# suutari/meterelf

Hardware: AMD Instinct MI355X
Metric: frames/sec (640x480), full pipeline, digits identical to the oracle (higher is better)
Workload: dtype u8; 1 GPU; Batch=1024 per GPU, full pipeline incl. TM_CCOEFF match + needle reading, 4 dials/frame, sample-images1 params, frames 480x640 synthesised from the readable fixtures (shift +-8, noise sigma 2), 4 distinct batches in rotation (3.77 GB of frames per GPU); global_batch=1024, parallelism=dp1, frames_read_ok_batch0=1023

## Files before the change

meterelf_amd/csrc/k_dials.hip:

```cpp
#include <limits.h>
#include <stdlib.h>

#include "melf_device.h"
#include "melf_internal.h"

namespace melf {

__device__ inline double py_fmod(double a, double b)
{
    double m = fmod(a, b);
    if (m != 0.0) {
        if ((b < 0) != (m < 0)) m += b;
    } else {
        m = copysign(0.0, b);
    }
    return m;
}

__device__ inline bool angle_by_vector(double x, double y, double& out)
{
    if (y == 0) {
        if (x > 0) { out = 0.25; return true; }
        if (x < 0) { out = 0.75; return true; }
        return false;
    }
    const double at = atan(x / y) / (2 * 3.141592653589793);
    const double v = -at + (y > 0 ? 0.5 : 0.0);
    double m = v - trunc(v);
    if (m != 0.0) { if (m < 0) m += 1.0; } else { m = 0.0; }
    out = m;
    return true;
}

__device__ inline double value_by_positions(double r4, double r3, double r2, double r1)
{
    int d3 = (int)r3 + ((py_fmod(r3, 1.0) > 0.55 && r4 <= 2) ? 1 : 0) - ((py_fmod(r3, 1.0) < 0.45 && r4 >= 8) ? 1 : 0);
    d3 = ((d3 % 10) + 10) % 10;
    int d2 = (int)r2 + ((py_fmod(r2, 1.0) > 0.55 && d3 <= 2) ? 1 : 0) - ((py_fmod(r2, 1.0) < 0.45 && d3 >= 8) ? 1 : 0);
    d2 = ((d2 % 10) + 10) % 10;
    int d1 = (int)r1 + ((py_fmod(r1, 1.0) > 0.55 && d2 <= 2) ? 1 : 0) - ((py_fmod(r1, 1.0) < 0.45 && d2 >= 8) ? 1 : 0);
    d1 = ((d1 % 10) + 10) % 10;
    return (d1 * 100.0) + (d2 * 10.0) + (d3 * 1.0) + r4 / 10.0;
}

struct Key {
    double a, d;
};
__device__ inline bool key_lt(const Key& p, const Key& q) { return p.a < q.a || (p.a == q.a && p.d < q.d); }
__device__ inline void wave_min_max_key(const Key& lo, const Key& hi, Key& klo, Key& khi)
{
    klo.a = wave_min_f64(lo.a);
    khi.a = wave_max_f64(hi.a);
    const uint64_t blo = __builtin_amdgcn_ballot_w64(lo.a == klo.a), bhi = __builtin_amdgcn_ballot_w64(hi.a == khi.a);
    if (__popcll(blo) == 1 && __popcll(bhi) == 1) {
        const int jl = __builtin_ctzll(blo), jh = __builtin_ctzll(bhi);
        const uint64_t dl = __double_as_longlong(lo.d), dh = __double_as_longlong(hi.d);
        klo.d = __longlong_as_double((uint64_t)(uint32_t)__builtin_amdgcn_readlane((int)(uint32_t)dl, jl) |
                                     ((uint64_t)(uint32_t)__builtin_amdgcn_readlane((int)(uint32_t)(dl >> 32), jl) << 32));
        khi.d = __longlong_as_double((uint64_t)(uint32_t)__builtin_amdgcn_readlane((int)(uint32_t)dh, jh) |
                                     ((uint64_t)(uint32_t)__builtin_amdgcn_readlane((int)(uint32_t)(dh >> 32), jh) << 32));
    } else {
        klo.d = wave_min_f64(lo.a == klo.a ? lo.d : 1e300);
        khi.d = wave_max_f64(hi.a == khi.a ? hi.d : -1e300);
    }
}

template <class F>
__device__ inline void for_each_kept(uint64_t outer, int lane, int wx0, int wy0, double cx, double cy,
                                     bool have_mom, double mom, F&& fn)
{
    const double dy = (double)(wy0 + lane) - cy;
    uint64_t bits = outer;
    while (bits) {
        const int x = __builtin_ctzll(bits);
        bits &= bits - 1;
        const double dx = (double)(wx0 + x) - cx;
        double a;
        if (angle_by_vector(dx, dy, a) && have_mom) {
            double dist = fabs(a - mom);
            const double dist2 = fabs(fabs(a - mom) - 1);
            if (dist2 < dist) dist = dist2;
            if (dist < 0.25) fn(a, dx * dx + dy * dy);
        }
    }
}

constexpr int DIAL_LIST_CAP = 768;
constexpr int RING_CAP = 512;
constexpr int RING_CAP_REGS = 1024;
constexpr int DIAL_LDS_BYTES = 5120;
static_assert(DIAL_LIST_CAP * 4 + DIAL_LIST_CAP * 2 <= 4608 && RING_CAP * 8 + RING_CAP * 2 <= DIAL_LDS_BYTES, "dial LDS layout");

__device__ __forceinline__ uint32_t load_px3(const uint8_t* p, const uint8_t* buffer_start)
{
    const uint32_t back = p == buffer_start ? 0u : 1u;
    uint32_t v;
    __builtin_memcpy(&v, p - back, 4);
    return v >> (8u * back);
}

struct PxColumn {
    const uint8_t* first;
    uint32_t shift;
};
__device__ __forceinline__ PxColumn px_column(const uint8_t* col, const uint8_t* buffer_start)
{
    const bool at_start = col == buffer_start;
    return PxColumn{at_start ? col : col - 1, at_start ? 0u : 8u};
}
__device__ __forceinline__ uint32_t load_px3_row(const PxColumn& c, size_t row_off)
{
    asm("" : "+s"(row_off));
    uint32_t v;
    __builtin_memcpy(&v, c.first + row_off, 4);
    return v >> c.shift;
}

typedef unsigned short u16x2v __attribute__((ext_vector_type(2)));
typedef uint32_t u32x4v __attribute__((ext_vector_type(4)));
__device__ __forceinline__ uint32_t pk_max_u16(uint32_t a, uint32_t b)
{
    return __builtin_bit_cast(uint32_t, __builtin_elementwise_max(__builtin_bit_cast(u16x2v, a), __builtin_bit_cast(u16x2v, b)));
}
__device__ __forceinline__ uint32_t pk_min_u16(uint32_t a, uint32_t b)
{
    return __builtin_bit_cast(uint32_t, __builtin_elementwise_min(__builtin_bit_cast(u16x2v, a), __builtin_bit_cast(u16x2v, b)));
}
__device__ __forceinline__ uint32_t pk_add_u16(uint32_t a, uint32_t b)
{
    return __builtin_bit_cast(uint32_t, (u16x2v)(__builtin_bit_cast(u16x2v, a) + __builtin_bit_cast(u16x2v, b)));
}
__device__ __forceinline__ uint32_t pk_sub_u16(uint32_t a, uint32_t b)
{
    return __builtin_bit_cast(uint32_t, (u16x2v)(__builtin_bit_cast(u16x2v, a) - __builtin_bit_cast(u16x2v, b)));
}
__device__ __forceinline__ uint32_t pk_mul_u16(uint32_t a, uint32_t b)
{
    return __builtin_bit_cast(uint32_t, (u16x2v)(__builtin_bit_cast(u16x2v, a) * __builtin_bit_cast(u16x2v, b)));
}

__device__ __forceinline__ void write_record(melf_result* __restrict__ out, int lane, int status, int mx, int my, float mv, int failed_dial,
                                             uint32_t unreadable, double value, double pos_lane, double angle_lane)
{
    if (lane < MELF_MAX_DIALS) {
        out->pos[lane] = pos_lane;
        out->angle[lane] = angle_lane;
    }
    if (lane == 0) {
        out->status = status;
        out->match_x = mx; out->match_y = my;
        out->failed_dial = failed_dial;
        out->unreadable_mask = unreadable;
        out->match_val = mv;
        out->value = value;
    }
}
static_assert(sizeof(melf_result) == 24 + 16 * MELF_MAX_DIALS + 8, "melf_result has padding: write_record must fill it");

#ifdef MELF_DIALS_STAMP
__device__ uint64_t g_dials_stamps[8 * 8192];
extern "C" __attribute__((visibility("default"))) int melf_debug_dials_stamps(uint64_t* out, int nwaves)
{
    return hipMemcpyFromSymbol(out, HIP_SYMBOL(g_dials_stamps), sizeof(uint64_t) * 8 * (size_t)(nwaves < 8192 ? nwaves : 8192)) == hipSuccess ? 0 : -1;
}
__device__ uint64_t g_dials_real[8 * 8192];
extern "C" __attribute__((visibility("default"))) int melf_debug_dials_real(uint64_t* out, int nwaves)
{
    return hipMemcpyFromSymbol(out, HIP_SYMBOL(g_dials_real), sizeof(uint64_t) * 8 * (size_t)(nwaves < 8192 ? nwaves : 8192)) == hipSuccess ? 0 : -1;
}
__device__ uint64_t g_dials_fine[16 * 8192];
extern "C" __attribute__((visibility("default"))) int melf_debug_dials_fine(uint64_t* out, int nwaves)
{
    return hipMemcpyFromSymbol(out, HIP_SYMBOL(g_dials_fine), sizeof(uint64_t) * 16 * (size_t)(nwaves < 8192 ? nwaves : 8192)) == hipSuccess ? 0 : -1;
}
#define FSTAMPD(k) do { if (lane == 0 && (int)(blockIdx.x * (blockDim.x >> 6) + wv) < 8192) g_dials_fine[16 * (blockIdx.x * (blockDim.x >> 6) + wv) + (k)] = __builtin_amdgcn_s_memtime(); } while (0)
#define DSTAMP(k) do { if (lane == 0 && (int)(blockIdx.x * (blockDim.x >> 6) + wv) < 8192) { \
        g_dials_stamps[8 * (blockIdx.x * (blockDim.x >> 6) + wv) + (k)] = __builtin_amdgcn_s_memtime(); \
        if ((k) < 6) g_dials_real[8 * (blockIdx.x * (blockDim.x >> 6) + wv) + (k)] = __builtin_amdgcn_s_memrealtime(); \
        if ((k) == 0) { uint32_t hw_; asm volatile("s_getreg_b32 %0, hwreg(HW_REG_HW_ID)" : "=s"(hw_)); uint32_t xc_; asm volatile("s_getreg_b32 %0, hwreg(HW_REG_XCC_ID)" : "=s"(xc_)); \
                        g_dials_real[8 * (blockIdx.x * (blockDim.x >> 6) + wv) + 6] = hw_; g_dials_real[8 * (blockIdx.x * (blockDim.x >> 6) + wv) + 7] = xc_ & 15u; } } } while (0)
#else
#define DSTAMP(k) do { } while (0)
#define FSTAMPD(k) do { } while (0)
#endif

constexpr int DIALS_VGPRS = 64;
template <int PB>
__device__ __forceinline__ uint32_t load_px(const uint8_t* p, const uint8_t* buffer_start)
{
    if constexpr (PB == 4) return *(const uint32_t*)p;
    else return load_px3(p, buffer_start);
}
template <int PB>
__device__ __forceinline__ PxColumn px_column_of(const uint8_t* col, const uint8_t* buffer_start)
{
    if constexpr (PB == 4) return PxColumn{col, 0u};
    else return px_column(col, buffer_start);
}

template <bool FROM_HLS, int NR>
__global__ __launch_bounds__(64 * MELF_MAX_DIALS, 4) __attribute__((amdgpu_num_vgpr(DIALS_VGPRS))) void k_dials(DialsSrc src, melf_params P,
                                                              const DialGeom* __restrict__ geom,
                                                              const uint64_t* __restrict__ rowmasks,
                                                              const MatchPartial* __restrict__ partials,
                                                              int nparts, int rw, melf_result* __restrict__ results)
{
    constexpr int PB = 3;
    constexpr bool RT_ORDER = false;
    const uint32_t bsel = 0u;
#include "k_dials_body.inc"
}

template <int BPP, int NR>
__global__ __launch_bounds__(64 * MELF_MAX_DIALS, 4) __attribute__((amdgpu_num_vgpr(DIALS_VGPRS))) void k_needles(DialsSrc src, melf_params P,
                                                                const DialGeom* __restrict__ geom,
                                                                const uint64_t* __restrict__ rowmasks,
                                                                const MatchPartial* __restrict__ partials,
                                                                int nparts, int rw, melf_result* __restrict__ results, int swap_rb)
{
    constexpr bool FROM_HLS = false;
    constexpr int PB = BPP;
    constexpr bool RT_ORDER = true;
    const uint32_t bsel = swap_rb ? 0x00020002u : 0u;
#include "k_dials_body.inc"
}

#define MELF_YUV_BODY
template <bool PLANAR, int NR>
__global__ __launch_bounds__(64 * MELF_MAX_DIALS, 4) __attribute__((amdgpu_num_vgpr(DIALS_VGPRS))) void k_yneedle(DialsSrc src, YuvPlanes yuv, YuvMatrix ymat, melf_params P,
                                                                const DialGeom* __restrict__ geom,
                                                                const uint64_t* __restrict__ rowmasks,
                                                                const MatchPartial* __restrict__ partials,
                                                                int nparts, int rw, melf_result* __restrict__ results)
{
    constexpr bool FROM_HLS = false;
    constexpr int PB = 4;
    constexpr bool RT_ORDER = false;
    const uint32_t bsel = 0u;
#include "k_dials_body.inc"
}
#undef MELF_YUV_BODY

#define MELF_P422_BODY
template <int NR>
__global__ __launch_bounds__(64 * MELF_MAX_DIALS, 4) __attribute__((amdgpu_num_vgpr(DIALS_VGPRS))) void k_p422_needle(DialsSrc src, uint32_t psel, YuvMatrix ymat, melf_params P,
                                                                const DialGeom* __restrict__ geom,
                                                                const uint64_t* __restrict__ rowmasks,
                                                                const MatchPartial* __restrict__ partials,
                                                                int nparts, int rw, melf_result* __restrict__ results)
{
    constexpr bool FROM_HLS = false;
    constexpr int PB = 4;
    constexpr bool RT_ORDER = false;
    const uint32_t bsel = 0u;
#include "k_dials_body.inc"
}
#undef MELF_P422_BODY

#define MELF_PLANAR_BODY
template <int NR>
__global__ __launch_bounds__(64 * MELF_MAX_DIALS, 4) __attribute__((amdgpu_num_vgpr(DIALS_VGPRS))) void k_planar_needle(DialsSrc src, PlanarPlanes planes, melf_params P,
                                                                const DialGeom* __restrict__ geom,
                                                                const uint64_t* __restrict__ rowmasks,
                                                                const MatchPartial* __restrict__ partials,
                                                                int nparts, int rw, melf_result* __restrict__ results)
{
    constexpr bool FROM_HLS = false;
    constexpr int PB = 4;
    constexpr bool RT_ORDER = false;
    const uint32_t bsel = 0u;
#include "k_dials_body.inc"
}
#undef MELF_PLANAR_BODY

void launch_dials(const DialsSrc& src, int pix, int n, const melf_params& P, const DialGeom* d_geom,
                  const uint64_t* d_rowmasks, const MatchPartial* d_partials, int nparts, int rw,
                  melf_result* d_results, hipStream_t stream, int ws_max, const YuvPlanes* yuv, const PlanarPlanes* planes,
                  const YuvMatrix* ymat)
{
    dim3 grid(n), block(64 * P.ndials);
    const size_t shmem = (size_t)P.ndials * DIAL_LDS_BYTES;
    const int nr = ws_max <= 32 ? 32 : (ws_max <= 40 ? 40 : (ws_max <= 48 ? 48 : (ws_max <= 52 ? 52 : (ws_max <= 56 ? 56 : 64))));
#define MELF_DIALS_LAUNCH(HLS, NRV) \
    hipLaunchKernelGGL((k_dials<HLS, NRV>), grid, block, shmem, stream, src, P, d_geom, d_rowmasks, d_partials, nparts, rw, d_results)
#define MELF_DIALS_NR(HLS)                                   \
    switch (nr) {                                            \
        case 32: MELF_DIALS_LAUNCH(HLS, 32); break;          \
        case 40: MELF_DIALS_LAUNCH(HLS, 40); break;          \
        case 48: MELF_DIALS_LAUNCH(HLS, 48); break;          \
        case 52: MELF_DIALS_LAUNCH(HLS, 52); break;          \
        case 56: MELF_DIALS_LAUNCH(HLS, 56); break;          \
        default: MELF_DIALS_LAUNCH(HLS, 64); break;          \
    }
#define MELF_NEEDLES_LAUNCH(BPP, NRV)                                                                                          \
    hipLaunchKernelGGL((k_needles<BPP, NRV>), grid, block, shmem, stream, src, P, d_geom, d_rowmasks, d_partials, nparts, rw, d_results, \
                       swap_rb)
#define MELF_NEEDLES_NR(BPP)                                 \
    switch (nr) {                                            \
        case 32: MELF_NEEDLES_LAUNCH(BPP, 32); break;        \
        case 40: MELF_NEEDLES_LAUNCH(BPP, 40); break;        \
        case 48: MELF_NEEDLES_LAUNCH(BPP, 48); break;        \
        case 52: MELF_NEEDLES_LAUNCH(BPP, 52); break;        \
        case 56: MELF_NEEDLES_LAUNCH(BPP, 56); break;        \
        default: MELF_NEEDLES_LAUNCH(BPP, 64); break;        \
    }
#define MELF_YNEEDLE_LAUNCH(PL, NRV) \
    hipLaunchKernelGGL((k_yneedle<PL, NRV>), grid, block, shmem, stream, src, *yuv, *ymat, P, d_geom, d_rowmasks, d_partials, nparts, rw, d_results)
#define MELF_YNEEDLE_NR(PL)                                  \
    switch (nr) {                                            \
        case 32: MELF_YNEEDLE_LAUNCH(PL, 32); break;         \
        case 40: MELF_YNEEDLE_LAUNCH(PL, 40); break;         \
        case 48: MELF_YNEEDLE_LAUNCH(PL, 48); break;         \
        case 52: MELF_YNEEDLE_LAUNCH(PL, 52); break;         \
        case 56: MELF_YNEEDLE_LAUNCH(PL, 56); break;         \
        default: MELF_YNEEDLE_LAUNCH(PL, 64); break;         \
    }
#define MELF_P422_NEEDLE_LAUNCH(NRV) \
    hipLaunchKernelGGL((k_p422_needle<NRV>), grid, block, shmem, stream, src, p422_sel(pix), *ymat, P, d_geom, d_rowmasks, d_partials, nparts, rw, d_results)
#define MELF_PLANAR_NEEDLE_LAUNCH(NRV) \
    hipLaunchKernelGGL((k_planar_needle<NRV>), grid, block, shmem, stream, src, *planes, P, d_geom, d_rowmasks, d_partials, nparts, rw, d_results)
    const int swap_rb = pix == MELF_PIX_RGB || pix == MELF_PIX_RGBA;
    if (pix == PIX_PLANAR) {
        switch (nr) {
            case 32: MELF_PLANAR_NEEDLE_LAUNCH(32); break;
            case 40: MELF_PLANAR_NEEDLE_LAUNCH(40); break;
            case 48: MELF_PLANAR_NEEDLE_LAUNCH(48); break;
            case 52: MELF_PLANAR_NEEDLE_LAUNCH(52); break;
            case 56: MELF_PLANAR_NEEDLE_LAUNCH(56); break;
            default: MELF_PLANAR_NEEDLE_LAUNCH(64); break;
        }
    }
    else if (pix_p422(pix)) {
        switch (nr) {
            case 32: MELF_P422_NEEDLE_LAUNCH(32); break;
            case 40: MELF_P422_NEEDLE_LAUNCH(40); break;
            case 48: MELF_P422_NEEDLE_LAUNCH(48); break;
            case 52: MELF_P422_NEEDLE_LAUNCH(52); break;
            case 56: MELF_P422_NEEDLE_LAUNCH(56); break;
            default: MELF_P422_NEEDLE_LAUNCH(64); break;
        }
    }
    else if (pix == PIX_NV12) { MELF_YNEEDLE_NR(false) }
    else if (pix == PIX_I420) { MELF_YNEEDLE_NR(true) }
    else if (pix == PIX_PLANE) { MELF_DIALS_NR(true) }
    else if (pix == MELF_PIX_BGR) { MELF_DIALS_NR(false) }
    else if (pix == MELF_PIX_RGB) { MELF_NEEDLES_NR(3) }
    else { MELF_NEEDLES_NR(4) }
#undef MELF_PLANAR_NEEDLE_LAUNCH
#undef MELF_P422_NEEDLE_LAUNCH
#undef MELF_YNEEDLE_NR
#undef MELF_YNEEDLE_LAUNCH
#undef MELF_NEEDLES_NR
#undef MELF_NEEDLES_LAUNCH
#undef MELF_DIALS_NR
#undef MELF_DIALS_LAUNCH
}

}
```

meterelf_amd/csrc/k_dials_body.inc:

```
    [[maybe_unused]] const uint32_t csel = bsel ? 0x0c000102u : 0x0c020100u;
    auto bgr = [&](uint32_t px) -> uint32_t {
        if constexpr (RT_ORDER) return __builtin_amdgcn_perm(0u, px, csel);
        else return px;
    };
    __shared__ int s_status[MELF_MAX_DIALS];
    __shared__ double s_pos[MELF_MAX_DIALS], s_angle[MELF_MAX_DIALS];
    extern __shared__ __attribute__((aligned(16))) uint8_t s_dyn[];

    const int f = blockIdx.x;
    const int lane = threadIdx.x & 63, wv = threadIdx.x >> 6;
    const int d = wv;
    DSTAMP(0);
    const uint8_t* frame = src.base + (size_t)f * src.frame_stride;
    uint8_t* const lds = s_dyn + (size_t)wv * DIAL_LDS_BYTES;
    uint32_t* const list_px = (uint32_t*)lds;
    uint16_t* const list_pos = (uint16_t*)(lds + 3072);
    double* const s_ra_d = (double*)lds;
    uint16_t* const ring_list = (uint16_t*)(lds + 4096);
    uint32_t* const mask_d = (uint32_t*)(lds + 4608);

    int mx = 0, my = 0;
    float mv = 0.f;
    if (!FROM_HLS) {
        float bv = 0.f;
        int bi = INT_MAX;
        for (int k = lane; k < nparts; k += 64) {
            const MatchPartial p = partials[(size_t)f * nparts + k];
            if (p.idx != INT_MAX && (bi == INT_MAX || p.val > bv || (p.val == bv && p.idx < bi))) { bv = p.val; bi = p.idx; }
        }
        {
            auto fold = [&](float ov, int oi) {
                if (oi != INT_MAX && (bi == INT_MAX || ov > bv || (ov == bv && oi < bi))) { bv = ov; bi = oi; }
            };
#define MELF_PFOLD(CTRL, RM, BM) \
            fold(__int_as_float(dpp_i32<CTRL, RM, BM>(0, __float_as_int(bv))), dpp_i32<CTRL, RM, BM>(INT_MAX, bi));
            MELF_PFOLD(0x111, 0xf, 0xf) MELF_PFOLD(0x112, 0xf, 0xf) MELF_PFOLD(0x114, 0xf, 0xe) MELF_PFOLD(0x118, 0xf, 0xc)
            MELF_PFOLD(0x142, 0xa, 0xf) MELF_PFOLD(0x143, 0xc, 0xf)
#undef MELF_PFOLD
            bv = __int_as_float(__builtin_amdgcn_readlane(__float_as_int(bv), 63));
            bi = __builtin_amdgcn_readlane(bi, 63);
        }
        mv = bv;
        const int mi = bi;
        mx = mi % rw;
        my = mi / rw;
        if ((double)mv < P.match_threshold) {
            if (wv == 0) write_record(results + f, lane, MELF_FRAME_DIALS_NOT_FOUND, mx, my, mv, -1, 0u, 0.0, 0.0, 0.0);
            return;
        }
    }

    DSTAMP(1);
    const DialGeom G = geom[d];
    const melf_dial D = P.dial[d];
    const int wx0 = __builtin_amdgcn_readfirstlane(G.wx0), wy0 = __builtin_amdgcn_readfirstlane(G.wy0), ws = __builtin_amdgcn_readfirstlane(G.ws);
    FSTAMPD(8);

    const int Xl = wx0 + lane;
    const bool colvalid = lane < ws && Xl >= 0 && Xl < P.tw;
    const int Xc = min(max(wx0 + min(lane, ws - 1), 0), P.tw - 1);
    const int ylast = ws - 1;
    const bool tail = !FROM_HLS && hls_scalar_tail(mx + Xl, src.crop_cols);
    const size_t rstride = FROM_HLS ? (size_t)P.tw * 3 : (size_t)src.row_stride;
#ifdef MELF_YUV_BODY
    const int fx_m = src.x0 + mx, fy_m = src.y0 + my;
    const int cp_u = __builtin_amdgcn_readfirstlane(yuv.c_pitch);
    const uint8_t* const uplane = frame + (size_t)yuv.u_off;
    const uint8_t* const vplane = frame + (size_t)yuv.v_off;
    auto yuv_px = [&](int X, int Y) -> uint32_t {
        const int fx = fx_m + X, fy = fy_m + Y;
        const size_t co = (size_t)(fy >> 1) * (size_t)cp_u + (size_t)(PLANAR ? fx >> 1 : fx & ~1);
        const int yv = frame[(size_t)fy * rstride + (size_t)fx];
        return yuv_bgr(yv, yuv_chroma<false>(uplane[co], vplane[co], ymat), ymat);
    };
#elif defined(MELF_P422_BODY)
    const int fx_m = src.x0 + mx, fy_m = src.y0 + my;
    auto yuv_px = [&](int X, int Y) -> uint32_t {
        const int fx = fx_m + X, fy = fy_m + Y;
        const uint32_t c = __builtin_amdgcn_perm(0u, *(const uint32_t*)(frame + (size_t)fy * rstride + (size_t)(fx >> 1) * 4), psel);
        return yuv_bgr((int)((fx & 1 ? c >> 16 : c) & 255u), yuv_chroma<false>((int)((c >> 8) & 255u), (int)(c >> 24), ymat), ymat);
    };
#elif defined(MELF_PLANAR_BODY)
    const int fx_m = src.x0 + mx, fy_m = src.y0 + my;
    const uint8_t* const bplane = frame + (size_t)planes.b_off;
    const uint8_t* const gplane = frame + (size_t)planes.g_off;
    const uint8_t* const rplane = frame + (size_t)planes.r_off;
    auto planar_px = [&](int X, int Y) -> uint32_t {
        const size_t o = (size_t)(fy_m + Y) * rstride + (size_t)(fx_m + X);
        return (uint32_t)bplane[o] | (uint32_t)gplane[o] << 8 | (uint32_t)rplane[o] << 16;
    };
#else
    const uint8_t* const origin = FROM_HLS ? frame : frame + (size_t)(src.y0 + my) * src.row_stride + (size_t)(src.x0 + mx) * PB;
#endif
    const int coreX = G.core_x - 2 + lane % 5, coreY = G.core_y - 2 + (lane < 25 ? lane / 5 : 0);
    const bool corevalid = lane < 25 && coreX >= 0 && coreX < P.tw && coreY >= 0 && coreY < P.th;
#if defined(MELF_YUV_BODY) || defined(MELF_P422_BODY)
    const uint32_t corepx = yuv_px(min(max(coreX, 0), P.tw - 1), min(max(coreY, 0), P.th - 1));
#elif defined(MELF_PLANAR_BODY)
    const uint32_t corepx = planar_px(min(max(coreX, 0), P.tw - 1), min(max(coreY, 0), P.th - 1));
#else
    const uint32_t corepx = bgr(load_px<PB>(origin + (size_t)min(max(coreY, 0), P.th - 1) * rstride + (size_t)min(max(coreX, 0), P.tw - 1) * PB, src.base));
    const PxColumn pcol = px_column_of<PB>(origin + (size_t)Xc * PB, src.base);
#endif
    const int th1 = __builtin_amdgcn_readfirstlane(P.th - 1);
    const int rs_u = __builtin_amdgcn_readfirstlane((int)rstride);
    constexpr int NG = NR / 4;
    static_assert(NR % 4 == 0, "window rows come in groups of four");
    const int rg = lane >> 4, pc = lane & 15;
    const int npiece = (ws + 3) >> 2;
    const uint8_t* const buf_end = src.base + src.readable;
#ifdef MELF_YUV_BODY
    (void)buf_end;
    const int xlim = (src.x0 + src.crop_cols + 1) & ~1;
    const bool quads = wx0 >= 0 && wx0 + 4 * npiece <= P.tw && xlim >= 8;
    const int fx0 = fx_m + wx0 + 4 * min(pc, npiece - 1);
    const int cstart = PLANAR ? min(fx0 >> 1, (xlim >> 1) - 4) : min(fx0 & ~1, xlim - 8);
    const uint32_t cshift = (uint32_t)((PLANAR ? fx0 >> 1 : fx0 & ~1) - cstart) * 8u;
    const bool fodd = fx0 & 1;
    auto yuv_quad = [&](const u32x4v r) -> u32x4v {
        uint32_t cu, cv;
        if constexpr (PLANAR) {
            cu = r.y >> cshift; cv = r.z >> cshift;
        } else {
            const uint64_t c = (((uint64_t)r.z << 32) | r.y) >> cshift;
            const uint32_t lo = (uint32_t)c, hi = (uint32_t)(c >> 32);
            cu = __builtin_amdgcn_perm(hi, lo, 0x0c040200u); cv = __builtin_amdgcn_perm(hi, lo, 0x0c050301u);
        }
        const YuvChroma c0 = yuv_chroma<false>(cu & 255, cv & 255, ymat), c1 = yuv_chroma<false>((cu >> 8) & 255, (cv >> 8) & 255, ymat),
                        c2 = yuv_chroma<false>((cu >> 16) & 255, (cv >> 16) & 255, ymat);
        u32x4v o;
        o.x = yuv_bgr(r.x & 255, c0, ymat);
        o.y = yuv_bgr((r.x >> 8) & 255, fodd ? c1 : c0, ymat);
        o.z = yuv_bgr((r.x >> 16) & 255, c1, ymat);
        o.w = yuv_bgr(r.x >> 24, fodd ? c2 : c1, ymat);
        return o;
    };
#elif defined(MELF_P422_BODY)
    (void)buf_end;
    const int mlim = (src.x0 + src.crop_cols + 1) >> 1;
    const bool quads = wx0 >= 0 && wx0 + 4 * npiece <= P.tw && mlim >= 3;
    const int fx0 = fx_m + wx0 + 4 * min(pc, npiece - 1);
    const int mstart = min(fx0 >> 1, mlim - 3);
    const bool mshifted = (fx0 >> 1) != mstart;
    const bool fodd = fx0 & 1;
    auto yuv_quad = [&](const u32x4v r) -> u32x4v {
        const uint32_t ma = __builtin_amdgcn_perm(0u, mshifted ? r.y : r.x, psel), mb = __builtin_amdgcn_perm(0u, mshifted ? r.z : r.y, psel),
                       mc = __builtin_amdgcn_perm(0u, r.z, psel);
        const YuvChroma c0 = yuv_chroma<false>((int)((ma >> 8) & 255u), (int)(ma >> 24), ymat), c1 = yuv_chroma<false>((int)((mb >> 8) & 255u), (int)(mb >> 24), ymat),
                        c2 = yuv_chroma<false>((int)((mc >> 8) & 255u), (int)(mc >> 24), ymat);
        const uint32_t y4 = __builtin_amdgcn_perm(mb, ma, 0x06040200u);
        const uint32_t yd = fodd ? __builtin_amdgcn_perm(mc, y4, 0x04030201u) : y4;
        u32x4v o;
        o.x = yuv_bgr((int)(yd & 255u), c0, ymat);
        o.y = yuv_bgr((int)((yd >> 8) & 255u), fodd ? c1 : c0, ymat);
        o.z = yuv_bgr((int)((yd >> 16) & 255u), c1, ymat);
        o.w = yuv_bgr((int)(yd >> 24), fodd ? c2 : c1, ymat);
        return o;
    };
#elif defined(MELF_PLANAR_BODY)
    (void)buf_end;
    const bool quads = wx0 >= 0 && wx0 + 4 * npiece <= P.tw;
    const int fx0 = fx_m + wx0 + 4 * min(pc, npiece - 1);
    auto planar_quad = [&](const u32x4v r) -> u32x4v {
        const uint32_t t01 = __builtin_amdgcn_perm(r.y, r.x, 0x05010400u), t23 = __builtin_amdgcn_perm(r.y, r.x, 0x07030602u);
        u32x4v o;
        o.x = __builtin_amdgcn_perm(r.z, t01, 0x0c040100u);
        o.y = __builtin_amdgcn_perm(r.z, t01, 0x0c050302u);
        o.z = __builtin_amdgcn_perm(r.z, t23, 0x0c060100u);
        o.w = __builtin_amdgcn_perm(r.z, t23, 0x0c070302u);
        return o;
    };
#else
    const bool quads = !FROM_HLS && ((uintptr_t)src.base & 3) == 0 && wx0 >= 0 && wx0 + 4 * npiece <= P.tw &&
                       origin + (size_t)th1 * rstride + (size_t)(wx0 + 4 * npiece) * PB + (PB == 4 ? 0 : 4) <= buf_end;
#endif
    u32x4v raw[NG];
    uint32_t mshift = 0;
#ifdef MELF_YUV_BODY
    if (quads) {
#pragma unroll
        for (int g = 0; g < NG; ++g) {
            const int fy = fy_m + min(max(wy0 + min(4 * g + rg, ylast), 0), th1);
            uint32_t yd;
            __builtin_memcpy(&yd, frame + (size_t)fy * (size_t)rs_u + (size_t)fx0, 4);
            const size_t co = (size_t)(fy >> 1) * (size_t)cp_u + (size_t)cstart;
            if constexpr (PLANAR) {
                uint32_t ud, vd;
                __builtin_memcpy(&ud, uplane + co, 4);
                __builtin_memcpy(&vd, vplane + co, 4);
                raw[g] = u32x4v{yd, ud, vd, 0u};
            } else {
                uint32_t cd[2];
                __builtin_memcpy(cd, uplane + co, 8);
                raw[g] = u32x4v{yd, cd[0], cd[1], 0u};
            }
        }
    }
#elif defined(MELF_P422_BODY)
    if (quads) {
#pragma unroll
        for (int g = 0; g < NG; ++g) {
            const int fy = fy_m + min(max(wy0 + min(4 * g + rg, ylast), 0), th1);
            uint32_t md[3];
            __builtin_memcpy(md, (const uint32_t*)(frame + (size_t)fy * (size_t)rs_u) + mstart, 12);
            raw[g] = u32x4v{md[0], md[1], md[2], 0u};
        }
    }
#elif defined(MELF_PLANAR_BODY)
    if (quads) {
#pragma unroll
        for (int g = 0; g < NG; ++g) {
            const int fy = fy_m + min(max(wy0 + min(4 * g + rg, ylast), 0), th1);
            const size_t o = (size_t)fy * (size_t)rs_u + (size_t)fx0;
            uint32_t bd, gd, rd;
            __builtin_memcpy(&bd, bplane + o, 4);
            __builtin_memcpy(&gd, gplane + o, 4);
            __builtin_memcpy(&rd, rplane + o, 4);
            raw[g] = u32x4v{bd, gd, rd, 0u};
        }
    }
#else
    if (quads) {
        const uint8_t* const lane0 = origin + (size_t)(wx0 + 4 * min(pc, npiece - 1)) * PB;
#pragma unroll
        for (int g = 0; g < NG; ++g) {
            const int Y = min(max(wy0 + min(4 * g + rg, ylast), 0), th1);
            const uint8_t* const a = lane0 + (size_t)Y * (size_t)rs_u;
            if constexpr (PB == 4) {
                raw[g] = *(const u32x4v*)a;
            } else {
                mshift |= ((uint32_t)(uintptr_t)a & 3u) << (2 * g);
                raw[g] = *(const u32x4v*)((uintptr_t)a & ~(uintptr_t)3);
            }
        }
    }
#endif
    __builtin_amdgcn_sched_barrier(0);
    FSTAMPD(9);
#ifdef MELF_DIALS_STAMP
    asm volatile("; colour core here" :: "v"(corepx) : "memory");
    FSTAMPD(10);
#endif

    int sh = 0, sl = 0, ss = 0, cnt = 0;
    if (corevalid) {
        if (FROM_HLS) { sh = corepx & 255; sl = (corepx >> 8) & 255; ss = (corepx >> 16) & 255; }
        else hls_pixel(corepx & 255, (corepx >> 8) & 255, (corepx >> 16) & 255, hls_scalar_tail(mx + coreX, src.crop_cols), P.hue_shift, sh, sl, ss);
        cnt = 1;
    }
    sh = wave_sum_i32(sh); sl = wave_sum_i32(sl); ss = wave_sum_i32(ss); cnt = wave_sum_i32(cnt);
    const double inv = cnt ? 1.0 / (double)cnt : 0.0;
    const int ch = (int)rint((double)sh * inv), cl = (int)rint((double)sl * inv), cs = (int)rint((double)ss * inv);
    const int loh = max(ch - D.range_h, 0), hih = min(ch + D.range_h, 255);
    const int lol = max(cl - D.range_l, 0), hil = min(cl + D.range_l, 255);
    const int los = max(cs - D.range_s, 0), his = min(cs + D.range_s, 255);

    DSTAMP(2);
    uint64_t m0 = 0, V = 0;
    auto exact_rows = [&]() {
        for (int yc = 0; yc < ws; yc += 16) {
            uint32_t pxe[16];
#pragma unroll
            for (int k = 0; k < 16; ++k) {
                const int Y = min(max(wy0 + min(yc + k, ylast), 0), th1);
#if defined(MELF_YUV_BODY) || defined(MELF_P422_BODY)
                pxe[k] = yuv_px(Xc, Y);
#elif defined(MELF_PLANAR_BODY)
                pxe[k] = planar_px(Xc, Y);
#else
                pxe[k] = bgr(load_px3_row(pcol, (size_t)((int64_t)Y * rs_u)));
#endif
            }
#pragma unroll
            for (int k = 0; k < 16; ++k) {
                const int y = yc + k, Y = wy0 + y;
                const bool valid = y < ws && colvalid && Y >= 0 && Y < P.th;
                bool in = false;
                if (valid) {
                    int H, L, S;
                    const uint32_t px = pxe[k];
                    if (FROM_HLS) { H = px & 255; L = (px >> 8) & 255; S = (px >> 16) & 255; }
                    else hls_pixel(px & 255, (px >> 8) & 255, (px >> 16) & 255, tail, P.hue_shift, H, L, S);
                    in = H >= loh && H <= hih && L >= lol && L <= hil && S >= los && S <= his;
                }
                const uint64_t b = __builtin_amdgcn_ballot_w64(in), vb = __builtin_amdgcn_ballot_w64(valid);
                if (lane == y) { m0 = b; V = vb; }
            }
        }
    };
    if (FROM_HLS) {
        exact_rows();
    } else {
        int total = 0;
        const uint64_t colb = __builtin_amdgcn_ballot_w64(colvalid);
        const uint32_t LO2 = (uint32_t)max(2 * lol - 1, 0) * 0x00010001u, HI2 = (uint32_t)(2 * hil + 1) * 0x00010001u;
        const uint32_t SLO = (uint32_t)max(los - 1, 0) * 0x00010001u, SHI = (uint32_t)(his + 1) * 0x00010001u;
        const int xleft = ws - 4 * pc;
        const uint64_t xm[4] = {__builtin_amdgcn_ballot_w64(0 < xleft), __builtin_amdgcn_ballot_w64(1 < xleft),
                                __builtin_amdgcn_ballot_w64(2 < xleft), __builtin_amdgcn_ballot_w64(3 < xleft)};
        if (quads) {
#pragma unroll
            for (int g = 0; g < NG; ++g) {
#if defined(MELF_YUV_BODY) || defined(MELF_P422_BODY)
                raw[g] = yuv_quad(raw[g]);
#elif defined(MELF_PLANAR_BODY)
                raw[g] = planar_quad(raw[g]);
#endif
                uint32_t e0 = 0, e1 = 0, e2 = 0;
                if constexpr (PB == 3) {
                    const uint32_t ms = (mshift >> (2 * g)) & 3u;
                    e0 = __builtin_amdgcn_alignbyte(raw[g].y, raw[g].x, ms);
                    e1 = __builtin_amdgcn_alignbyte(raw[g].z, raw[g].y, ms);
                    e2 = __builtin_amdgcn_alignbyte(raw[g].w, raw[g].z, ms);
                }
                const int y = 4 * g + rg, Y = wy0 + y;
                const uint64_t rowb = __builtin_amdgcn_ballot_w64((y < ws) & (Y >= 0) & (Y < P.th));
                const uint32_t sb = RT_ORDER ? bsel : 0u;
#pragma unroll
                for (int h = 0; h < 2; ++h) {
                    uint32_t B2, G2, R2;
                    if constexpr (PB == 4) {
                        const uint32_t lo = h ? raw[g].z : raw[g].x, hi = h ? raw[g].w : raw[g].y;
                        B2 = __builtin_amdgcn_perm(hi, lo, 0x0c040c00u + sb);
                        G2 = __builtin_amdgcn_perm(hi, lo, 0x0c050c01u);
                        R2 = __builtin_amdgcn_perm(hi, lo, 0x0c060c02u - sb);
                    } else {
                        B2 = h ? __builtin_amdgcn_perm(e2, e1, 0x0c050c02u + sb) : __builtin_amdgcn_perm(e1, e0, 0x0c030c00u + sb);
                        G2 = h ? __builtin_amdgcn_perm(e2, e1, 0x0c060c03u) : __builtin_amdgcn_perm(e1, e0, 0x0c040c01u);
                        R2 = h ? __builtin_amdgcn_perm(e2, e1, 0x0c070c04u - sb) : __builtin_amdgcn_perm(e1, e0, 0x0c050c02u - sb);
                    }
                    const uint32_t vmax = pk_max_u16(pk_max_u16(B2, G2), R2), vmin = pk_min_u16(pk_min_u16(B2, G2), R2);
                    const uint32_t sum = pk_add_u16(vmax, vmin), diff = pk_sub_u16(vmax, vmin);
                    const uint32_t den = pk_min_u16(sum, pk_sub_u16(0x01fe01feu, sum));
                    const uint32_t lbad = pk_min_u16(pk_max_u16(sum, LO2), HI2) ^ sum;
                    const uint32_t a = pk_mul_u16(diff, 0x00ff00ffu);
                    const uint32_t sbad = pk_min_u16(pk_max_u16(a, pk_mul_u16(den, SLO)), pk_mul_u16(den, SHI)) ^ a;
                    const uint32_t bad = lbad | sbad;
#pragma unroll
                    for (int q = 0; q < 2; ++q) {
                        const int j = 2 * h + q;
                        const uint64_t cb = __builtin_amdgcn_ballot_w64(q ? bad < 0x10000u : (bad & 0xffffu) == 0u) & rowb & xm[j];
                        if (cb) {
                            const int slot = total + (int)__builtin_amdgcn_mbcnt_hi((uint32_t)(cb >> 32), __builtin_amdgcn_mbcnt_lo((uint32_t)cb, 0u));
                            const bool cand = (cb >> lane) & 1ull;
                            if (cand && slot < DIAL_LIST_CAP) {
                                list_pos[slot] = (uint16_t)(y << 6 | (4 * pc + j));
                                if constexpr (PB == 4)
                                    list_px[slot] = bgr(j == 0 ? raw[g].x : (j == 1 ? raw[g].y : (j == 2 ? raw[g].z : raw[g].w)));
                                else
                                    list_px[slot] = bgr(j == 0 ? e0 : (j == 1 ? __builtin_amdgcn_alignbyte(e1, e0, 3) : (j == 2 ? __builtin_amdgcn_alignbyte(e2, e1, 2) : e2 >> 8)));
                            }
                            total += __popcll(cb);
                        }
                    }
                }
            }
        } else {
            total = DIAL_LIST_CAP + 1;
        }
        V = (lane < ws && wy0 + lane >= 0 && wy0 + lane < P.th && lane < NR) ? colb : 0ull;
        DSTAMP(6);
#ifdef MELF_DIALS_STAMP
        if (lane == 0 && (int)(blockIdx.x * (blockDim.x >> 6) + wv) < 8192) g_dials_real[8 * (blockIdx.x * (blockDim.x >> 6) + wv) + 6] |= (uint64_t)total << 32;
#endif
        if (total > DIAL_LIST_CAP) {
            exact_rows();
        } else {
            mask_d[lane] = 0;
            mask_d[64 + lane] = 0;
            DSTAMP(7);
            for (int t = lane; t < total; t += 64) {
                const int e = list_pos[t], y = e >> 6, x = e & 63;
                const uint32_t px = list_px[t];
                int H, L, S;
                hls_pixel(px & 255, (px >> 8) & 255, (px >> 16) & 255, hls_scalar_tail(mx + wx0 + x, src.crop_cols), P.hue_shift, H, L, S);
                if (H >= loh && H <= hih && L >= lol && L <= hil && S >= los && S <= his)
                    atomicOr(&mask_d[2 * y + (x >> 5)], 1u << (x & 31));
            }
            m0 = (uint64_t)mask_d[2 * lane] | ((uint64_t)mask_d[2 * lane + 1] << 32);
        }
    }

    DSTAMP(3);
    const uint64_t hz = m0 | (m0 << 1) | (m0 >> 1);
    const uint64_t dil = (hz | row_up(hz, lane, 0) | row_down(hz, lane, 0)) | ~V;
    const uint64_t he = dil & ((dil << 1) | 1ull) & ((dil >> 1) | (1ull << 63));
    const uint64_t mde = he & row_up(he, lane, ~0ull) & row_down(he, lane, ~0ull) & V;

    const uint64_t disk = rowmasks[((size_t)d * 3 + 0) * 64 + lane];
    const uint64_t annulus = rowmasks[((size_t)d * 3 + 1) * 64 + lane];
    const uint64_t outside0 = rowmasks[((size_t)d * 3 + 2) * 64 + lane];
    const uint64_t M = mde & disk;
    FSTAMPD(0);

    int status = 0;
    double pos = 0.0, angle = 0.0;
    if (__builtin_amdgcn_ballot_w64(M != 0) == 0) {
        status = 1;
    } else {
        uint64_t bestF = 0;
        int best2 = -1, ncomp = 0;
        auto label = [&](const uint64_t Gs) {
            uint64_t rem = Gs;
            bestF = 0; best2 = -1; ncomp = 0;
            for (;;) {
                const uint64_t rowsb = __builtin_amdgcn_ballot_w64(rem != 0);
                if (rowsb == 0) break;
                const int r0 = __builtin_ctzll(rowsb);
                const uint64_t rv = (uint64_t)(uint32_t)__builtin_amdgcn_readlane((int)(uint32_t)rem, r0) |
                                    ((uint64_t)(uint32_t)__builtin_amdgcn_readlane((int)(uint32_t)(rem >> 32), r0) << 32);
                const int b0 = __builtin_ctzll(rv);
                uint64_t s = (lane == r0) ? (1ull << b0) : 0ull;
                for (;;) {
                    const uint64_t h3 = s | (s << 1) | (s >> 1);
                    const uint64_t n1 = (h3 | row_up(h3, lane, 0) | row_down(h3, lane, 0)) & Gs;
                    const uint64_t g3 = n1 | (n1 << 1) | (n1 >> 1);
                    const uint64_t n2 = (g3 | row_up(g3, lane, 0) | row_down(g3, lane, 0)) & Gs;
                    const bool ch2 = n2 != n1;
                    s = n2;
                    if (__builtin_amdgcn_ballot_w64(ch2) == 0) break;
                }
                const uint64_t a = s, b = row_down(s, lane, 0), a1 = a >> 1, b1 = b >> 1;
                const int c = 2 * __builtin_popcountll(a & a1 & b & b1) + __builtin_popcountll(a & a1 & b & ~b1) +
                              __builtin_popcountll(a & a1 & ~b & b1) + __builtin_popcountll(a & ~a1 & b & b1) +
                              __builtin_popcountll(~a & a1 & b & b1);
                const int area2 = wave_sum_i32(c);
                if (area2 > best2) { best2 = area2; bestF = s; }
                rem &= ~s;
                ++ncomp;
            }
        };
        int euler4, isolated;
        {
            const uint64_t a = M, b = row_down(M, lane, 0), a1 = a >> 1, b1 = b >> 1;
            const uint64_t odd = a ^ a1 ^ b ^ b1;
            const uint64_t three = odd & ((a & a1) | (b & b1));
            const uint64_t diag = (a & b1 & ~a1 & ~b) | (a1 & b & ~a & ~b1);
            euler4 = wave_sum_i32(__builtin_popcountll(odd) - 2 * __builtin_popcountll(three) - 2 * __builtin_popcountll(diag));
            const uint64_t up = row_up(M, lane, 0);
            const uint64_t nb = (a << 1) | a1 | up | (up << 1) | (up >> 1) | b | (b << 1) | b1;
            isolated = wave_sum_i32(__builtin_popcountll(a & ~nb));
        }
        bool holes = euler4 - 4 * isolated <= 0;
        if (!holes) {
            label(M);
            holes = 4 * ncomp != euler4;
        }
        FSTAMPD(1);
#ifdef MELF_DIALS_STAMP
        if (lane == 0 && (int)(blockIdx.x * (blockDim.x >> 6) + wv) < 8192) {
            g_dials_fine[16 * (blockIdx.x * (blockDim.x >> 6) + wv) + 12] = (uint64_t)(uint32_t)euler4;
            g_dials_fine[16 * (blockIdx.x * (blockDim.x >> 6) + wv) + 13] = (uint64_t)(uint32_t)ncomp;
            g_dials_fine[16 * (blockIdx.x * (blockDim.x >> 6) + wv) + 14] = (uint64_t)(uint32_t)isolated;
        }
#endif
        if (holes) {
            const uint64_t freeb = ~M;
            uint64_t o = outside0;
            for (;;) {
                const uint64_t n1 = o | ((((o << 1) | (o >> 1)) | row_up(o, lane, ~0ull) | row_down(o, lane, ~0ull)) & freeb);
                const uint64_t n2 = n1 | ((((n1 << 1) | (n1 >> 1)) | row_up(n1, lane, ~0ull) | row_down(n1, lane, ~0ull)) & freeb);
                const bool ch2 = n2 != n1;
                o = n2;
                if (__builtin_amdgcn_ballot_w64(ch2) == 0) break;
            }
            label(~o);
        }
        DSTAMP(4);
        const uint64_t N = (best2 > 200 ? bestF : M) & disk;
        const uint64_t outer = N & annulus;

        const double cx = D.cx, cy = D.cy;
        double sx = 0.0, sy = 0.0;
        FSTAMPD(2);
        {
            const double dy = (double)(wy0 + lane) - cy;
            const double ty = (dy < 0 ? -1.0 : 1.0) * (dy * dy);
            const double* const mt = (const double*)(rowmasks + (size_t)P.ndials * 3 * 64) + (size_t)d * 2048;
            double part[8];
#pragma unroll
            for (int b = 0; b < 8; ++b) part[b] = mt[b * 256 + (int)((N >> (8 * b)) & 255)];
            sx = ((part[0] + part[1]) + (part[2] + part[3])) + ((part[4] + part[5]) + (part[6] + part[7]));
            sy = ty * (double)__builtin_popcountll(N);
        }
        sx = wave_sum_f64(sx);
        sy = wave_sum_f64(sy);
        FSTAMPD(3);
        const double msign = D.negative_momentum ? -1.0 : 1.0;
        double mom = 0.0;
        const bool have_mom = angle_by_vector(msign * sx, msign * sy, mom);
        FSTAMPD(4);

        const int rmine = __popcll(outer);
        const int rincl = wave_scan_i32(rmine);
        const int rtotal = __builtin_amdgcn_readlane(rincl, 63);
#ifdef MELF_DIALS_STAMP
        if (lane == 0 && (int)(blockIdx.x * (blockDim.x >> 6) + wv) < 8192) g_dials_real[8 * (blockIdx.x * (blockDim.x >> 6) + wv) + 7] |= (uint64_t)rtotal << 32;
#endif
        if (rtotal <= RING_CAP) {
            uint16_t* list = ring_list;
            double* ra = s_ra_d;
            {
                int at = rincl - rmine;
                uint64_t bits = outer;
                while (bits) {
                    const int x = __builtin_ctzll(bits);
                    bits &= bits - 1;
                    list[at++] = (uint16_t)(lane << 6 | x);
                }
            }
            FSTAMPD(5);
            auto ring_d2 = [&](int e) {
                const double dx = (double)(wx0 + (e & 63)) - cx, dy = (double)(wy0 + (e >> 6)) - cy;
                return dx * dx + dy * dy;
            };
            int nk = 0;
            double mina = 1e300;
            for (int t = lane; t < rtotal; t += 64) {
                const int e = list[t];
                const double dx = (double)(wx0 + (e & 63)) - cx, dy = (double)(wy0 + (e >> 6)) - cy;
                double a, keep = __builtin_nan("");
                if (angle_by_vector(dx, dy, a) && have_mom) {
                    double dist = fabs(a - mom);
                    const double dist2 = fabs(fabs(a - mom) - 1);
                    if (dist2 < dist) dist = dist2;
                    if (dist < 0.25) { keep = a; ++nk; if (a < mina) mina = a; }
                }
                ra[t] = keep;
            }
            nk = wave_sum_i32(nk);
            mina = wave_min_f64(mina);
            if (nk == 0) {
                status = 2;
            } else {
                FSTAMPD(6);
                const int cut = nk >= 5 ? min(2, (nk - 3) / 2) : 0;
                const Key PINF = {1e300, 1e300}, NINF = {-1e300, -1e300};
                Key klo = NINF, khi = PINF;
                if (cut > 0) {
                    Key l1 = PINF, l2 = PINF, h1 = NINF, h2 = NINF;
                    for (int t = lane; t < rtotal; t += 64) {
                        const double a = ra[t];
                        if (a != a) continue;
                        Key k;
                        k.a = fabs(a - mina) < 0.75 ? a : a - 1;
                        k.d = ring_d2(list[t]);
                        if (key_lt(k, l1)) { l2 = l1; l1 = k; } else if (key_lt(k, l2)) { l2 = k; }
                        if (key_lt(h1, k)) { h2 = h1; h1 = k; } else if (key_lt(h2, k)) { h2 = k; }
                    }
                    for (int c2 = 0; c2 < cut; ++c2) {
                        wave_min_max_key(l1, h1, klo, khi);
                        if (l1.a == klo.a && l1.d == klo.d) { l1 = l2; l2 = PINF; }
                        if (h1.a == khi.a && h1.d == khi.d) { h1 = h2; h2 = NINF; }
                    }
                }
                FSTAMPD(7);
                double sad = 0.0, sd = 0.0;
                for (int t = lane; t < rtotal; t += 64) {
                    const double a = ra[t];
                    if (a != a) continue;
                    Key k;
                    k.a = fabs(a - mina) < 0.75 ? a : a - 1;
                    k.d = ring_d2(list[t]);
                    if (cut == 0 || (key_lt(klo, k) && key_lt(k, khi))) {
                        sad += k.a * k.d;
                        sd += k.d;
                    }
                }
                sad = wave_sum_f64(sad);
                sd = wave_sum_f64(sd);
                angle = sad / sd;
                const double fixed = angle - (D.angle_of_zero / 360.0);
                pos = py_fmod(10.0 * fixed, 10.0);
            }
        } else if (rtotal <= RING_CAP_REGS) {
            uint16_t* list = (uint16_t*)lds;
            {
                int at = rincl - rmine;
                uint64_t bits = outer;
                while (bits) {
                    const int x = __builtin_ctzll(bits);
                    bits &= bits - 1;
                    list[at++] = (uint16_t)(lane << 6 | x);
                }
            }
            auto ring_d2 = [&](int e) {
                const double dx = (double)(wx0 + (e & 63)) - cx, dy = (double)(wy0 + (e >> 6)) - cy;
                return dx * dx + dy * dy;
            };
            constexpr int NJ = RING_CAP_REGS / 64;
            double ang[NJ];
            int nk = 0;
            double mina = 1e300;
#pragma unroll
            for (int j = 0; j < NJ; ++j) {
                double keep = __builtin_nan("");
                if (64 * j < rtotal) {
                    const int t = lane + 64 * j;
                    if (t < rtotal) {
                        const int e = list[t];
                        const double dx = (double)(wx0 + (e & 63)) - cx, dy = (double)(wy0 + (e >> 6)) - cy;
                        double a;
                        if (angle_by_vector(dx, dy, a) && have_mom) {
                            double dist = fabs(a - mom);
                            const double dist2 = fabs(fabs(a - mom) - 1);
                            if (dist2 < dist) dist = dist2;
                            if (dist < 0.25) { keep = a; ++nk; if (a < mina) mina = a; }
                        }
                    }
                }
                ang[j] = keep;
            }
            nk = wave_sum_i32(nk);
            mina = wave_min_f64(mina);
            if (nk == 0) {
                status = 2;
            } else {
                const int cut = nk >= 5 ? min(2, (nk - 3) / 2) : 0;
                const Key PINF = {1e300, 1e300}, NINF = {-1e300, -1e300};
                Key klo = NINF, khi = PINF;
                if (cut > 0) {
                    Key l1 = PINF, l2 = PINF, h1 = NINF, h2 = NINF;
#pragma unroll
                    for (int j = 0; j < NJ; ++j) {
                        const double a = ang[j];
                        if (a != a) continue;
                        Key k;
                        k.a = fabs(a - mina) < 0.75 ? a : a - 1;
                        k.d = ring_d2(list[lane + 64 * j]);
                        if (key_lt(k, l1)) { l2 = l1; l1 = k; } else if (key_lt(k, l2)) { l2 = k; }
                        if (key_lt(h1, k)) { h2 = h1; h1 = k; } else if (key_lt(h2, k)) { h2 = k; }
                    }
                    for (int c2 = 0; c2 < cut; ++c2) {
                        wave_min_max_key(l1, h1, klo, khi);
                        if (l1.a == klo.a && l1.d == klo.d) { l1 = l2; l2 = PINF; }
                        if (h1.a == khi.a && h1.d == khi.d) { h1 = h2; h2 = NINF; }
                    }
                }
                double sad = 0.0, sd = 0.0;
#pragma unroll
                for (int j = 0; j < NJ; ++j) {
                    const double a = ang[j];
                    if (a != a) continue;
                    Key k;
                    k.a = fabs(a - mina) < 0.75 ? a : a - 1;
                    k.d = ring_d2(list[lane + 64 * j]);
                    if (cut == 0 || (key_lt(klo, k) && key_lt(k, khi))) {
                        sad += k.a * k.d;
                        sd += k.d;
                    }
                }
                sad = wave_sum_f64(sad);
                sd = wave_sum_f64(sd);
                angle = sad / sd;
                const double fixed = angle - (D.angle_of_zero / 360.0);
                pos = py_fmod(10.0 * fixed, 10.0);
            }
        } else {
            int nk = 0;
            double mina = 1e300;
            for_each_kept(outer, lane, wx0, wy0, cx, cy, have_mom, mom, [&](double a, double) {
                ++nk;
                if (a < mina) mina = a;
            });
            nk = wave_sum_i32(nk);
                mina = wave_min_f64(mina);
            if (nk == 0) {
                status = 2;
            } else {
                const int cut = nk >= 5 ? min(2, (nk - 3) / 2) : 0;
                const Key PINF = {1e300, 1e300}, NINF = {-1e300, -1e300};
                Key klo = NINF, khi = PINF;
                if (cut > 0) {
                    Key l1 = PINF, l2 = PINF, h1 = NINF, h2 = NINF;
                    for_each_kept(outer, lane, wx0, wy0, cx, cy, have_mom, mom, [&](double a, double dd) {
                        Key k;
                        k.a = fabs(a - mina) < 0.75 ? a : a - 1;
                        k.d = dd;
                        if (key_lt(k, l1)) { l2 = l1; l1 = k; } else if (key_lt(k, l2)) { l2 = k; }
                        if (key_lt(h1, k)) { h2 = h1; h1 = k; } else if (key_lt(h2, k)) { h2 = k; }
                    });
                    for (int c2 = 0; c2 < cut; ++c2) {
                        wave_min_max_key(l1, h1, klo, khi);
                        if (l1.a == klo.a && l1.d == klo.d) { l1 = l2; l2 = PINF; }
                        if (h1.a == khi.a && h1.d == khi.d) { h1 = h2; h2 = NINF; }
                    }
                }
                double sad = 0.0, sd = 0.0;
                for_each_kept(outer, lane, wx0, wy0, cx, cy, have_mom, mom, [&](double a, double dd) {
                    Key k;
                    k.a = fabs(a - mina) < 0.75 ? a : a - 1;
                    k.d = dd;
                    if (cut == 0 || (key_lt(klo, k) && key_lt(k, khi))) {
                        sad += k.a * dd;
                        sd += dd;
                    }
                });
                sad = wave_sum_f64(sad);
                sd = wave_sum_f64(sd);
                angle = sad / sd;
                const double fixed = angle - (D.angle_of_zero / 360.0);
                pos = py_fmod(10.0 * fixed, 10.0);
            }
        }
    }
    DSTAMP(5);
    if (lane == 0) { s_status[d] = status; s_pos[d] = pos; s_angle[d] = angle; }
    __syncthreads();

    if (wv == 0) {
        int st = MELF_FRAME_OK, failed = -1;
        uint32_t unread = 0;
        double value = 0.0;
        for (int k = 0; k < P.ndials; ++k)
            if (s_status[k] == 2) unread |= 1u << k;
        for (int k = 0; k < P.ndials; ++k)
            if (s_status[k] == 1) { st = MELF_FRAME_NEEDLE_CONTOURS_NOT_FOUND; failed = k; break; }
        if (st == MELF_FRAME_NEEDLE_CONTOURS_NOT_FOUND) {
            unread &= (1u << failed) - 1u;
        } else if (unread) {
            st = MELF_FRAME_ANGLE_UNDETERMINED;
        } else if (P.ndials == 4) {
            value = value_by_positions(s_pos[P.name_order[0]], s_pos[P.name_order[1]], s_pos[P.name_order[2]], s_pos[P.name_order[3]]);
        }
        const bool has = lane < P.ndials;
        write_record(results + f, lane, st, mx, my, mv, failed, unread, value, has ? s_pos[has ? lane : 0] : 0.0, has ? s_angle[has ? lane : 0] : 0.0);
    }
```

Measured before the change: 4.380 million frames/s.

## Replace per-quad ballot compaction with per-lane bitmasks and a wave scan

The candidate-pixel compaction used to issue a ballot, an mbcnt and scattered LDS stores for every row group and column. Now each lane builds a per-row-group bitmask of candidates, a single wave prefix scan assigns list offsets, and each lane writes its entries in one pass. The LDS list keeps only positions; the exact HLS check re-reads each pixel from global memory instead of a stored copy. This cuts ballot and LDS traffic in the hot loop, but adds scattered global reloads and an inline asm dependency.

```diff
diff --git a/meterelf_amd/csrc/k_dials.hip b/meterelf_amd/csrc/k_dials.hip
--- a/meterelf_amd/csrc/k_dials.hip
+++ b/meterelf_amd/csrc/k_dials.hip
@@ -89,7 +89,7 @@
 constexpr int RING_CAP = 512;
 constexpr int RING_CAP_REGS = 1024;
 constexpr int DIAL_LDS_BYTES = 5120;
-static_assert(DIAL_LIST_CAP * 4 + DIAL_LIST_CAP * 2 <= 4608 && RING_CAP * 8 + RING_CAP * 2 <= DIAL_LDS_BYTES, "dial LDS layout");
+static_assert(DIAL_LIST_CAP * 2 <= 4608 && RING_CAP * 8 + RING_CAP * 2 <= DIAL_LDS_BYTES, "dial LDS layout");
 
 __device__ __forceinline__ uint32_t load_px3(const uint8_t* p, const uint8_t* buffer_start)
 {
diff --git a/meterelf_amd/csrc/k_dials_body.inc b/meterelf_amd/csrc/k_dials_body.inc
--- a/meterelf_amd/csrc/k_dials_body.inc
+++ b/meterelf_amd/csrc/k_dials_body.inc
@@ -1,5 +1,5 @@
     [[maybe_unused]] const uint32_t csel = bsel ? 0x0c000102u : 0x0c020100u;
-    auto bgr = [&](uint32_t px) -> uint32_t {
+    [[maybe_unused]] auto bgr = [&](uint32_t px) -> uint32_t {
         if constexpr (RT_ORDER) return __builtin_amdgcn_perm(0u, px, csel);
         else return px;
     };
@@ -13,8 +13,7 @@
     DSTAMP(0);
     const uint8_t* frame = src.base + (size_t)f * src.frame_stride;
     uint8_t* const lds = s_dyn + (size_t)wv * DIAL_LDS_BYTES;
-    uint32_t* const list_px = (uint32_t*)lds;
-    uint16_t* const list_pos = (uint16_t*)(lds + 3072);
+    uint16_t* const list_pos = (uint16_t*)lds;
     double* const s_ra_d = (double*)lds;
     uint16_t* const ring_list = (uint16_t*)(lds + 4096);
     uint32_t* const mask_d = (uint32_t*)(lds + 4608);
@@ -291,14 +290,14 @@
     if (FROM_HLS) {
         exact_rows();
     } else {
-        int total = 0;
+        int total;
         const uint64_t colb = __builtin_amdgcn_ballot_w64(colvalid);
         const uint32_t LO2 = (uint32_t)max(2 * lol - 1, 0) * 0x00010001u, HI2 = (uint32_t)(2 * hil + 1) * 0x00010001u;
         const uint32_t SLO = (uint32_t)max(los - 1, 0) * 0x00010001u, SHI = (uint32_t)(his + 1) * 0x00010001u;
         const int xleft = ws - 4 * pc;
-        const uint64_t xm[4] = {__builtin_amdgcn_ballot_w64(0 < xleft), __builtin_amdgcn_ballot_w64(1 < xleft),
-                                __builtin_amdgcn_ballot_w64(2 < xleft), __builtin_amdgcn_ballot_w64(3 < xleft)};
         if (quads) {
+            static_assert(NG <= 16, "one bit per row group in a 16-bit half");
+            uint32_t nc[2] = {0u, 0u};
 #pragma unroll
             for (int g = 0; g < NG; ++g) {
 #if defined(MELF_YUV_BODY) || defined(MELF_P422_BODY)
@@ -313,8 +312,6 @@
                     e1 = __builtin_amdgcn_alignbyte(raw[g].z, raw[g].y, ms);
                     e2 = __builtin_amdgcn_alignbyte(raw[g].w, raw[g].z, ms);
                 }
-                const int y = 4 * g + rg, Y = wy0 + y;
-                const uint64_t rowb = __builtin_amdgcn_ballot_w64((y < ws) & (Y >= 0) & (Y < P.th));
                 const uint32_t sb = RT_ORDER ? bsel : 0u;
 #pragma unroll
                 for (int h = 0; h < 2; ++h) {
@@ -336,22 +333,30 @@
                     const uint32_t a = pk_mul_u16(diff, 0x00ff00ffu);
                     const uint32_t sbad = pk_min_u16(pk_max_u16(a, pk_mul_u16(den, SLO)), pk_mul_u16(den, SHI)) ^ a;
                     const uint32_t bad = lbad | sbad;
-#pragma unroll
-                    for (int q = 0; q < 2; ++q) {
-                        const int j = 2 * h + q;
-                        const uint64_t cb = __builtin_amdgcn_ballot_w64(q ? bad < 0x10000u : (bad & 0xffffu) == 0u) & rowb & xm[j];
-                        if (cb) {
-                            const int slot = total + (int)__builtin_amdgcn_mbcnt_hi((uint32_t)(cb >> 32), __builtin_amdgcn_mbcnt_lo((uint32_t)cb, 0u));
-                            const bool cand = (cb >> lane) & 1ull;
-                            if (cand && slot < DIAL_LIST_CAP) {
-                                list_pos[slot] = (uint16_t)(y << 6 | (4 * pc + j));
-                                if constexpr (PB == 4)
-                                    list_px[slot] = bgr(j == 0 ? raw[g].x : (j == 1 ? raw[g].y : (j == 2 ? raw[g].z : raw[g].w)));
-                                else
-                                    list_px[slot] = bgr(j == 0 ? e0 : (j == 1 ? __builtin_amdgcn_alignbyte(e1, e0, 3) : (j == 2 ? __builtin_amdgcn_alignbyte(e2, e1, 2) : e2 >> 8)));
-                            }
-                            total += __popcll(cb);
-                        }
+                    uint32_t nz;
+                    asm("v_pk_min_u16 %0, %1, %2" : "=v"(nz) : "v"(bad), "v"(0x00010001u));
+                    nc[h] |= nz << g;
+                }
+            }
+            FSTAMPD(11);
+            const int ya = max(-wy0, 0), yb = min(min(ws, P.th - wy0), NR);
+            const int glo = min((ya - rg + 3) >> 2, 16), ghi = max(yb - rg + 3, 0) >> 2;
+            const uint32_t rowm = ((1u << ghi) - 1u) & ~((1u << glo) - 1u);
+            const uint32_t c0 = ~nc[0] & ((0 < xleft ? rowm : 0u) | (1 < xleft ? rowm << 16 : 0u));
+            const uint32_t c1 = ~nc[1] & ((2 < xleft ? rowm : 0u) | (3 < xleft ? rowm << 16 : 0u));
+            const int mine = __popc(c0) + __popc(c1);
+            const int incl = wave_scan_i32(mine);
+            total = __builtin_amdgcn_readlane(incl, 63);
+            if (total <= DIAL_LIST_CAP) {
+                uint16_t* at = list_pos + (incl - mine);
+                const uint32_t pos0 = (uint32_t)(rg << 6 | 4 * pc);
+#pragma unroll
+                for (int j = 0; j < 4; ++j) {
+                    uint32_t bits = j & 1 ? (j & 2 ? c1 : c0) >> 16 : (j & 2 ? c1 : c0) & 0xffffu;
+                    while (bits) {
+                        const uint32_t g = (uint32_t)__builtin_ctz(bits);
+                        bits &= bits - 1u;
+                        *at++ = (uint16_t)(pos0 + (uint32_t)j + (g << 8));
                     }
                 }
             }
@@ -371,7 +376,13 @@
             DSTAMP(7);
             for (int t = lane; t < total; t += 64) {
                 const int e = list_pos[t], y = e >> 6, x = e & 63;
-                const uint32_t px = list_px[t];
+#if defined(MELF_YUV_BODY) || defined(MELF_P422_BODY)
+                const uint32_t px = yuv_px(wx0 + x, wy0 + y);
+#elif defined(MELF_PLANAR_BODY)
+                const uint32_t px = planar_px(wx0 + x, wy0 + y);
+#else
+                const uint32_t px = bgr(load_px<PB>(origin + (size_t)(wy0 + y) * rstride + (size_t)(wx0 + x) * PB, src.base));
+#endif
                 int H, L, S;
                 hls_pixel(px & 255, (px >> 8) & 255, (px >> 16) & 255, hls_scalar_tail(mx + wx0 + x, src.crop_cols), P.hue_shift, H, L, S);
                 if (H >= loh && H <= hih && L >= lol && L <= hil && S >= los && S <= his)
```

Result: no change. 4.365 million frames/s (-0.3%).
